# wavelab/libwave

Hardware: AMD Instinct MI355X
Metric: point-cloud registrations/sec (1M<->1M pts, ICP) (higher is better)
Workload: dtype f32

## Files before the change

include/wavematch.h:

```cpp
#ifndef WAVEMATCH_H
#define WAVEMATCH_H

#include <stddef.h>
#include <stdint.h>

#ifdef __cplusplus
extern "C" {
#endif

#define WM_OK 0
#define WM_NOT_CONVERGED 1
#define WM_TOO_FEW_CORRESPONDENCES 2
#define WM_ERR_ARG (-1)
#define WM_ERR_HIP (-2)
#define WM_ERR_RCCL (-3)
#define WM_ERR_STATE (-4)
#define WM_ERR_NOMEM (-5)

enum { WM_MEM_HOST = 0, WM_MEM_DEVICE = 1 };

typedef struct wm_ctx wm_ctx;

int wm_ctx_create(wm_ctx **out, int device);
void wm_ctx_destroy(wm_ctx *ctx);
// ... 33 lines not shown
    int nn_method;
    int carry_state;
    int profile;
    int normal_k;
    int reject;
    double reject_ratio;
    double reject_factor;
    int reject_min_corr;
} wm_icp_params;

typedef struct {
    int converged;
    int iterations;
    int state;
    int n_corr;
    double mse;
    double prev_mse;
    float align_ms;
    float nn_ms;
    float coarse_ms;
    float stats_ms;
    float solve_ms;
    int nn_launches;
    int nn_levels;
    uint64_t deferred;
    float grid_cell;
    int owned_violations;
    int cert_launches;
    float nn_cert_ms;
    float plan_ms;
    float compact_ms;
    float index_ms;
    float iter_ms;
    float allreduce_ms;
    unsigned n_tgt_local, n_src_local;
    int rccl_ranks;
    int shard_attempts;
    int late_iterations;
    int late_launches;
    float late_ms;
    int exchange_in_kernel;
    int n_matched;
    float reject_d2;
} wm_icp_stats;

void wm_icp_default_params(wm_icp_params *p);

int wm_icp_align(wm_ctx *ctx, const wm_icp_params *p, double T_out[16], wm_icp_stats *stats);

int wm_icp_match(wm_ctx *ctx, const void *ref, size_t n_ref, const void *target, size_t n_target,
                 size_t stride_bytes, int mem, const wm_icp_params *p, float res,
                 int multiscale_steps, double T_out[16], wm_icp_stats *stats);

#define WM_BATCH_LDS_TARGET_POINTS 10000
#define WM_BATCH_MAX_TARGET_POINTS 65535
typedef struct {
    const void *src;
    size_t n_src;
    const void *target;
    size_t n_target;
} wm_batch_item;
int wm_icp_batch_match(wm_ctx *ctx, const wm_batch_item *items, int n_items, size_t stride_bytes,
                       int mem, const wm_icp_params *p, float res, int multiscale_steps,
                       int with_info, double *T_out, double *info_out, wm_icp_stats *stats,
                       int *status);

int wm_voxel_downsample_batch(wm_ctx *ctx, const wm_batch_item *items, int n_items, size_t stride_bytes,
                              int mem, float leaf, float *out_xyz, size_t cap_points, size_t *n_out);

int wm_voxel_downsample(wm_ctx *ctx, const void *pts, size_t n, size_t stride_bytes, int mem,
                        float leaf, void *out, size_t out_stride, int out_mem, size_t cap,
                        size_t *n_out);

int wm_transform_cloud(wm_ctx *ctx, const void *pts, size_t n, size_t stride_bytes, int mem,
                       const double T[16], void *out, size_t out_stride, int out_mem);

enum { WM_INFO_LUM = 0, WM_INFO_CENSI = 1, WM_INFO_LUMOLD = 2 };
int wm_icp_info(wm_ctx *ctx, int method, const double T_result[16], double lin_covar,
                double ang_covar, double max_corr, double info[36], int *degenerate);

int wm_debug_copy_bandwidth(wm_ctx *ctx, size_t bytes, int reps, double *gb_per_s);
int wm_debug_bins_sum(const double *x, size_t n, const unsigned *perm, double *out, long long limbs_out[3]);
int wm_debug_sort_pairs(wm_ctx *ctx, const void *keys, int key_bytes, size_t n, unsigned bits, unsigned *values_out);
int wm_debug_knn(wm_ctx *ctx, int which, int k, int32_t *idx_out, float *d2_out);
int wm_set_option(wm_ctx *ctx, const char *name, double value);
int wm_debug_cert_log(wm_ctx *ctx, int iterations, unsigned *out, int cap);
int wm_debug_cert_prof(wm_ctx *ctx, unsigned long long *out, int cap);
int wm_debug_pub_log(wm_ctx *ctx, unsigned long long *out, int cap);
int wm_get_iteration_times(wm_ctx *ctx, float *nn_ms, int cap);

int wm_debug_solve_cycles(wm_ctx *ctx, unsigned long long out[8]);
int wm_debug_cost_log(wm_ctx *ctx, int iterations, unsigned *out, size_t cap);
int wm_debug_phase_log(wm_ctx *ctx, unsigned long long *out, int iterations);

int wm_get_correspondences(wm_ctx *ctx, int32_t *match_idx, float *d2, size_t cap);

int wm_nn_search(wm_ctx *ctx, const double T[16], double max_corr, int nn_method,
                 int32_t *match_idx, float *d2, size_t cap, float *kernel_ms);

int wm_estimate_normals(wm_ctx *ctx, int which, int k, void *normals_out, int out_mem);

#define WM_STATS_LEN 32
int wm_icp_stats_for(wm_ctx *ctx, const double T[16], int mode, double stats[WM_STATS_LEN]);

int wm_debug_rank_select(wm_ctx *ctx, const float *vals, size_t n, size_t rank, float *out);

typedef struct { int n_matched, n_kept; float threshold_d2; int all_kept; } wm_icp_reject_result;
int wm_icp_reject(wm_ctx *ctx, const double T[16], int mode, int reject, double ratio, double factor, int min_corr,
                  wm_icp_reject_result *res, unsigned char *kept_out, double stats_out[WM_STATS_LEN]);

int wm_umeyama_from_stats(const double stats[WM_STATS_LEN], double Tk_out[16]);
int wm_gn6_from_stats(const double stats[WM_STATS_LEN], double Tk_out[16]);

typedef struct {
    int corr_rand;
    int max_iter;
    double r_eps;
    double t_eps;
    double max_corr;
    double gicp_epsilon;
    int max_inner;
    int force_iterations;
    int objective;
    int reserved;
} wm_gicp_params;
#define WM_GICP_OBJECTIVE_PCL_SUMS 0
#define WM_GICP_OBJECTIVE_STATISTICS 1

typedef struct {
    int converged, iterations, n_corr, inner_total, evaluations;
    double f_final;
    float fdf_kernel_ms;
    int served_evaluations;
} wm_gicp_stats;

void wm_gicp_default_params(wm_gicp_params *p);
int wm_gicp_align(wm_ctx *ctx, const wm_gicp_params *p, double T_out[16], wm_gicp_stats *stats);
int wm_gicp_match(wm_ctx *ctx, const void *ref, size_t n_ref, const void *target, size_t n_target,
                  size_t stride_bytes, int mem, const wm_gicp_params *p, float res, double T_out[16],
                  wm_gicp_stats *stats);
int wm_set_source_filtered(wm_ctx *ctx, const void *pts, size_t n, size_t stride_bytes, int mem, float leaf);
int wm_set_target_filtered(wm_ctx *ctx, const void *pts, size_t n, size_t stride_bytes, int mem, float leaf);
#define WM_GICP_BATCH_MAX_POINTS 100000
int wm_gicp_batch_match(wm_ctx *ctx, const wm_batch_item *items, int n_items, size_t stride_bytes, int mem,
                        const wm_gicp_params *p, float res, double *T_out, wm_gicp_stats *stats, int *status,
                        float *kernel_ms);
int wm_gicp_eval(wm_ctx *ctx, const wm_gicp_params *p, const double T_pair[16], const double x[6],
                 double *f, double g[6], int *n_pairs);
int wm_gicp_covariances(wm_ctx *ctx, int k, double eps, double *cov_source, double *cov_target);

typedef struct {
    double res;
    double step_size;
    double t_eps;
    int max_iter;
    double outlier_ratio;
    int skip_line_search;
    int pcl_d1_sign;
    int force_iterations;
} wm_ndt_params;

typedef struct {
    int converged, iterations, n_voxels, evaluations;
    double score;
    float deriv_kernel_ms;
    int model_builds;
// ... 173 lines not shown
```

libwave_amd/capi.py:

```python
import ctypes as C
import os

import numpy as np

_HERE = os.path.dirname(os.path.abspath(__file__))
LIB_PATH = os.path.join(_HERE, "libwavematch_hip.so")

WM_OK, WM_NOT_CONVERGED, WM_TOO_FEW = 0, 1, 2
WM_ERR_ARG, WM_ERR_HIP, WM_ERR_RCCL, WM_ERR_STATE, WM_ERR_NOMEM = -1, -2, -3, -4, -5
WM_NDT_BATCH_MAX_POINTS = 200000
WM_GICP_BATCH_MAX_POINTS = 100000
WM_BATCH_LDS_TARGET_POINTS = 10000
WM_BATCH_MAX_TARGET_POINTS = 65535
WM_GROUND_BATCH_MAX_KEYS = 0xFFFFFFFF
WM_GROUND_BATCH_MAX_POINTS = 0x7FFFFFF0
WM_MEM_HOST, WM_MEM_DEVICE = 0, 1
WM_ICP_SVD, WM_ICP_GN6, WM_ICP_PLANE = 0, 1, 2
WM_REJECT_NONE, WM_REJECT_TRIMMED, WM_REJECT_MEDIAN = 0, 1, 2
WM_NN_AUTO, WM_NN_GRID, WM_NN_BRUTE = 0, 1, 2
WM_NN_WARM = 0x100
WM_INFO_LUM, WM_INFO_CENSI, WM_INFO_LUMOLD = 0, 1, 2
WM_STATS_LEN = 32
CONV_NAMES = {0: "NOT_CONVERGED", 1: "ITERATIONS", 2: "TRANSFORM", 3: "ABS_MSE", 4: "REL_MSE",
              5: "NO_CORRESPONDENCES", 6: "FORCED", 7: "DEGENERATE"}
# ... 156 lines not shown
        L.wm_debug_pub_log.argtypes = [C.c_void_p, C.POINTER(C.c_uint64), C.c_int]
        L.wm_cloud_sizes.argtypes = [C.c_void_p, C.POINTER(C.c_size_t), C.POINTER(C.c_size_t)]
        L.wm_icp_default_params.argtypes = [C.POINTER(IcpParams)]
        L.wm_icp_default_params.restype = None
        L.wm_icp_align.argtypes = [C.c_void_p, C.POINTER(IcpParams), _dp, C.POINTER(IcpStats)]
        L.wm_icp_match.argtypes = [C.c_void_p, C.c_void_p, C.c_size_t, C.c_void_p, C.c_size_t,
                                   C.c_size_t, C.c_int, C.POINTER(IcpParams), C.c_float, C.c_int,
                                   _dp, C.POINTER(IcpStats)]
        L.wm_icp_batch_match.argtypes = [C.c_void_p, C.POINTER(BatchItem), C.c_int, C.c_size_t, C.c_int,
                                         C.POINTER(IcpParams), C.c_float, C.c_int, C.c_int, _dp, _dp,
                                         C.POINTER(IcpStats), C.POINTER(C.c_int)]
        L.wm_gicp_batch_match.argtypes = [C.c_void_p, C.POINTER(BatchItem), C.c_int, C.c_size_t, C.c_int,
                                          C.POINTER(GicpParams), C.c_float, _dp, C.POINTER(GicpStats),
                                          C.POINTER(C.c_int), C.POINTER(C.c_float)]
        L.wm_ndt_batch_match.argtypes = [C.c_void_p, C.POINTER(BatchItem), C.c_int, C.c_size_t, C.c_int,
                                         C.POINTER(NdtParams), _dp, C.POINTER(NdtStats), C.POINTER(C.c_int),
                                         C.POINTER(C.c_float)]
        L.wm_voxel_downsample_batch.argtypes = [C.c_void_p, C.POINTER(BatchItem), C.c_int, C.c_size_t, C.c_int,
                                                C.c_float, _fp, C.c_size_t, C.POINTER(C.c_size_t)]
        L.wm_voxel_downsample.argtypes = [C.c_void_p, C.c_void_p, C.c_size_t, C.c_size_t, C.c_int,
                                          C.c_float, C.c_void_p, C.c_size_t, C.c_int, C.c_size_t,
                                          C.POINTER(C.c_size_t)]
        L.wm_transform_cloud.argtypes = [C.c_void_p, C.c_void_p, C.c_size_t, C.c_size_t, C.c_int,
                                         _dp, C.c_void_p, C.c_size_t, C.c_int]
        L.wm_icp_info.argtypes = [C.c_void_p, C.c_int, _dp, C.c_double, C.c_double, C.c_double, _dp,
                                  C.POINTER(C.c_int)]
        L.wm_ctx_set_stream.argtypes = [C.c_void_p, C.c_void_p, C.c_int]
        L.wm_icp_shard_begin.argtypes = [C.c_void_p, C.POINTER(IcpParams), C.c_double, C.c_double,
                                         C.c_size_t]
        L.wm_icp_shard_local_stats.argtypes = [C.c_void_p, C.c_void_p]
        L.wm_icp_shard_apply.argtypes = [C.c_void_p, C.c_void_p]
        L.wm_icp_shard_poll.argtypes = [C.c_void_p, C.POINTER(C.c_int), _dp, C.POINTER(IcpStats)]
        L.wm_host_icp_create.argtypes = [C.POINTER(C.c_void_p), C.POINTER(IcpParams), C.c_size_t]
        L.wm_host_icp_destroy.argtypes = [C.c_void_p]
        L.wm_host_icp_destroy.restype = None
        L.wm_host_icp_apply.argtypes = [C.c_void_p, _dp]
        L.wm_host_icp_get.argtypes = [C.c_void_p, C.POINTER(C.c_int), _dp, C.POINTER(IcpStats)]
        L.wm_gicp_default_params.argtypes = [C.POINTER(GicpParams)]
        L.wm_gicp_default_params.restype = None
        L.wm_gicp_align.argtypes = [C.c_void_p, C.POINTER(GicpParams), _dp, C.POINTER(GicpStats)]
        L.wm_gicp_match.argtypes = [C.c_void_p, C.c_void_p, C.c_size_t, C.c_void_p, C.c_size_t,
                                    C.c_size_t, C.c_int, C.POINTER(GicpParams), C.c_float, _dp,
                                    C.POINTER(GicpStats)]
        L.wm_gicp_eval.argtypes = [C.c_void_p, C.POINTER(GicpParams), _dp, _dp, _dp, _dp,
                                   C.POINTER(C.c_int)]
        L.wm_gicp_covariances.argtypes = [C.c_void_p, C.c_int, C.c_double, _dp, _dp]
        L.wm_ndt_default_params.argtypes = [C.POINTER(NdtParams)]
        L.wm_ndt_default_params.restype = None
        L.wm_ndt_align.argtypes = [C.c_void_p, C.POINTER(NdtParams), _dp, C.POINTER(NdtStats)]
        L.wm_ndt_derivatives.argtypes = [C.c_void_p, C.POINTER(NdtParams), _dp, _dp, _dp, _dp,
                                         C.POINTER(C.c_int)]
        L.wm_ndt_set_shard.argtypes = [C.c_void_p, C.c_int, C.c_int, ALLREDUCE_FN, C.c_void_p]
        L.wm_get_iteration_times.argtypes = [C.c_void_p, _fp, C.c_int]
        L.wm_comm_get_unique_id.argtypes = [C.c_void_p]
        L.wm_comm_init_rank.argtypes = [C.POINTER(C.c_void_p), C.c_int, C.c_void_p, C.c_int, C.c_int]
        L.wm_comm_init_all.argtypes = [C.POINTER(C.c_void_p), C.POINTER(C.c_int), C.c_int]
        L.wm_comm_init_local.argtypes = [C.POINTER(C.c_void_p), C.c_int, C.c_int]
        L.wm_comm_destroy.argtypes = [C.c_void_p]
        L.wm_comm_destroy.restype = None
        L.wm_comm_rank.argtypes = [C.c_void_p]
        L.wm_comm_allreduce_probe.argtypes = [C.c_void_p, C.c_void_p, C.c_int, _dp]
        L.wm_comm_world.argtypes = [C.c_void_p]
        L.wm_comm_mailboxes.argtypes = [C.c_void_p]
        L.wm_comm_set_exchange_timeout_ms.argtypes = [C.c_void_p, C.c_int]
        L.wm_icp_align_sharded.argtypes = [C.c_void_p, C.c_void_p, C.c_void_p, C.c_size_t, C.c_void_p,
                                           C.c_size_t, C.c_size_t, C.c_int, C.POINTER(IcpParams), _dp,
                                           C.POINTER(IcpStats)]
        L.wm_ndt_set_comm.argtypes = [C.c_void_p, C.c_void_p]
        L.wm_ndt_build_model.argtypes = [C.c_void_p, C.c_double]
        L.wm_set_source_filtered.argtypes = [C.c_void_p, C.c_void_p, C.c_size_t, C.c_size_t, C.c_int, C.c_float]
        L.wm_set_target_filtered.argtypes = [C.c_void_p, C.c_void_p, C.c_size_t, C.c_size_t, C.c_int, C.c_float]
        L.wm_multi_create.argtypes = [C.POINTER(C.c_void_p), C.POINTER(C.c_int), C.c_int, C.c_int]
        L.wm_multi_destroy.argtypes = [C.c_void_p]
        L.wm_multi_destroy.restype = None
        L.wm_multi_size.argtypes = [C.c_void_p]
        L.wm_multi_icp_align.argtypes = [C.c_void_p, C.c_void_p, C.c_size_t, C.c_void_p, C.c_size_t,
                                         C.c_size_t, C.POINTER(IcpParams), _dp, C.POINTER(IcpStats)]
        L.wm_multi_icp_match.argtypes = [C.c_void_p, C.c_void_p, C.c_size_t, C.c_void_p, C.c_size_t,
                                         C.c_size_t, C.POINTER(IcpParams), C.c_float, C.c_int, _dp, C.POINTER(IcpStats)]
        L.wm_multi_icp_info.argtypes = [C.c_void_p, C.c_int, _dp, C.c_double, C.c_double, C.c_double, _dp,
                                        C.POINTER(C.c_int)]
        L.wm_debug_solve_cycles.argtypes = [C.c_void_p, C.POINTER(C.c_uint64)]
        L.wm_debug_sort_pairs.argtypes = [C.c_void_p, C.c_void_p, C.c_int, C.c_size_t, C.c_uint, C.c_void_p]
        L.wm_debug_knn.argtypes = [C.c_void_p, C.c_int, C.c_int, _ip, _fp]
        L.wm_debug_cost_log.argtypes = [C.c_void_p, C.c_int, C.c_void_p, C.c_size_t]
        L.wm_debug_phase_log.argtypes = [C.c_void_p, C.c_void_p, C.c_int]
        L.wm_get_correspondences.argtypes = [C.c_void_p, _ip, _fp, C.c_size_t]
        L.wm_nn_search.argtypes = [C.c_void_p, _dp, C.c_double, C.c_int, _ip, _fp, C.c_size_t, _fp]
        L.wm_icp_stats_for.argtypes = [C.c_void_p, _dp, C.c_int, _dp]
        L.wm_debug_rank_select.argtypes = [C.c_void_p, _fp, C.c_size_t, C.c_size_t, _fp]
        L.wm_icp_reject.argtypes = [C.c_void_p, _dp, C.c_int, C.c_int, C.c_double, C.c_double, C.c_int,
                                    C.POINTER(IcpRejectResult), C.c_void_p, _dp]
        L.wm_estimate_normals.argtypes = [C.c_void_p, C.c_int, C.c_int, C.c_void_p, C.c_int]
        L.wm_umeyama_from_stats.argtypes = [_dp, _dp]
        L.wm_gn6_from_stats.argtypes = [_dp, _dp]
        L.wm_ground_default_params.argtypes = [C.POINTER(GroundParams)]
        L.wm_ground_default_params.restype = None
        L.wm_ground_segment.argtypes = [C.c_void_p, C.c_void_p, C.c_size_t, C.c_size_t, C.c_int,
                                        C.POINTER(GroundParams), C.c_int, C.c_void_p, C.c_size_t, C.c_int,
                                        C.POINTER(C.c_size_t), C.c_void_p, C.POINTER(GroundStats)]
        L.wm_ground_segment_batch.argtypes = [C.c_void_p, C.POINTER(GroundScan), C.c_int, C.c_size_t, C.c_int,
                                              C.POINTER(GroundParams), C.c_int, C.c_void_p, C.c_size_t, C.c_void_p,
                                              C.c_size_t, C.c_int, C.POINTER(C.c_size_t), C.c_void_p,
                                              C.POINTER(GroundStats), C.POINTER(C.c_float)]
        L.wm_outlier_default_params.argtypes = [C.POINTER(OutlierParams)]
        L.wm_outlier_default_params.restype = None
        L.wm_outlier_filter.argtypes = [C.c_void_p, C.c_void_p, C.c_size_t, C.c_size_t, C.c_int, C.POINTER(OutlierParams),
                                        C.c_void_p, C.c_size_t, C.c_int, C.POINTER(C.c_size_t), C.c_void_p, C.c_void_p,
                                        C.c_void_p, C.POINTER(OutlierStats)]
        L.wm_cluster_default_params.argtypes = [C.POINTER(ClusterParams)]
        L.wm_cluster_default_params.restype = None
        L.wm_cluster_extract.argtypes = [C.c_void_p, C.c_void_p, C.c_size_t, C.c_size_t, C.c_int, C.POINTER(ClusterParams),
                                         C.c_void_p, C.c_void_p, C.c_size_t, C.c_void_p, C.c_size_t, C.c_int,
                                         C.POINTER(C.c_size_t), C.POINTER(C.c_size_t), C.POINTER(ClusterStats)]
        L.wm_cluster_extract_batch.argtypes = [C.c_void_p, C.POINTER(ClusterScan), C.c_int, C.c_size_t, C.c_int,
                                               C.POINTER(ClusterParams), C.c_void_p, C.c_void_p, C.c_size_t, C.c_void_p,
                                               C.c_size_t, C.c_void_p, C.c_size_t, C.c_int, C.POINTER(C.c_size_t),
                                               C.POINTER(C.c_size_t), C.POINTER(ClusterStats), C.POINTER(C.c_float)]
        _LIB = L
    return _LIB


def declared_symbols(header=None):
    import re
    inc = os.path.join(os.path.dirname(_HERE), "include")
    names = []
    for fn in sorted(os.listdir(inc)):
        if not fn.endswith(".h"):
            continue
        txt = open(os.path.join(inc, fn)).read()
        txt = re.sub(r"/\*.*?\*/", "", txt, flags=re.S)
        names += re.findall(r"\b(wm_[a-z0-9_]+)\s*\(", txt)
    return sorted(set(names))


def gicp_params(**kw):
    p = GicpParams()
    lib().wm_gicp_default_params(C.byref(p))
    for k, v in kw.items():
        if not hasattr(p, k):
            raise AttributeError(k)
        setattr(p, k, v)
    return p


def ndt_params(**kw):
    p = NdtParams()
    lib().wm_ndt_default_params(C.byref(p))
    for k, v in kw.items():
        if not hasattr(p, k):
            raise AttributeError(k)
        setattr(p, k, v)
    return p


def icp_params(**kw):
    p = IcpParams()
    lib().wm_icp_default_params(C.byref(p))
    for k, v in kw.items():
        if not hasattr(p, k):
            raise AttributeError(k)
        setattr(p, k, v)
    return p


def ground_params(params=None, **kw):
# ... 571 lines not shown

    def set_stream(self, stream_ptr, external=True):
        self._check(lib().wm_ctx_set_stream(self._h, C.c_void_p(stream_ptr), int(external)),
                    "wm_ctx_set_stream")

    def shard_begin(self, params, x_lo, x_hi, expect_owned_total=0):
        self._check(lib().wm_icp_shard_begin(self._h, C.byref(params), float(x_lo), float(x_hi),
                                             int(expect_owned_total)), "wm_icp_shard_begin")

    def shard_local_stats(self, dev_ptr):
        self._check(lib().wm_icp_shard_local_stats(self._h, C.c_void_p(dev_ptr)),
                    "wm_icp_shard_local_stats")

    def shard_apply(self, dev_ptr):
        self._check(lib().wm_icp_shard_apply(self._h, C.c_void_p(dev_ptr)), "wm_icp_shard_apply")

    def shard_poll(self):
        done = C.c_int(0)
        T = np.zeros((4, 4), np.float64)
        s = IcpStats()
        rc = self._check(lib().wm_icp_shard_poll(self._h, C.byref(done), T.ctypes.data_as(_dp),
                                                 C.byref(s)), "wm_icp_shard_poll")
        d = self._stats_dict(rc, T, s)
        d["T"] = T
        d["done"] = bool(done.value)
        return d

    def icp_align_sharded(self, comm, ref, target, params=None, **kw):
        p = params or icp_params(**kw)
        rp, rn, rs, rm, k1 = _cloud_arg(ref)
        tp, tn, ts, tm, k2 = _cloud_arg(target)
        if rs != ts or rm != tm:
            raise WmError("ref and target must share stride and memory space")
        T = np.zeros((4, 4), np.float64)
        s = IcpStats()
        rc = self._check(lib().wm_icp_align_sharded(self._h, comm.handle if comm is not None else None,
                                                    C.c_void_p(rp), rn, C.c_void_p(tp), tn, rs, rm,
                                                    C.byref(p), T.ctypes.data_as(_dp), C.byref(s)),
                         "wm_icp_align_sharded")
        return self._sharded_dict(rc, T, s)

    @staticmethod
    def _sharded_dict(rc, T, s):
        d = Context._stats_dict(rc, T, s)
        d["owned_violations"] = s.owned_violations
        for k in ("plan_ms", "compact_ms", "index_ms", "iter_ms", "allreduce_ms", "n_tgt_local", "n_src_local",
                  "rccl_ranks", "shard_attempts", "exchange_in_kernel"):
            d[k] = getattr(s, k)
        return d

    def allreduce_probe(self, comm, reps=50):
        out = C.c_double(0)
        self._check(lib().wm_comm_allreduce_probe(self._h, comm.handle, int(reps), C.byref(out)),
                    "wm_comm_allreduce_probe")
        return out.value

    def ndt_set_comm(self, comm):
        self._check(lib().wm_ndt_set_comm(self._h, comm.handle if comm is not None else None),
                    "wm_ndt_set_comm")

    def cost_log_arm(self, iterations):
        self._check(lib().wm_debug_cost_log(self._h, iterations, None, 0), "wm_debug_cost_log")

    def cost_log_fetch(self, iterations, n):
        buf = np.zeros((iterations, n), np.uint32)
        k = lib().wm_debug_cost_log(self._h, iterations, buf.ctypes.data_as(C.c_void_p), buf.size)
        if k < 0:
            raise WmError("wm_debug_cost_log: %d" % k)
        return buf[:k]

    def phase_log_fetch(self, iterations):
        buf = np.zeros((iterations, 8), np.uint64)
        k = lib().wm_debug_phase_log(self._h, buf.ctypes.data_as(C.c_void_p), iterations)
        return buf[:max(k, 0)]

    def sort_pairs(self, keys, bits):
        keys = np.ascontiguousarray(keys)
        assert keys.dtype in (np.uint32, np.uint64) and keys.ndim == 1
        out = np.zeros(keys.shape[0], np.uint32)
        self._check(lib().wm_debug_sort_pairs(self._h, keys.ctypes.data, keys.dtype.itemsize, keys.shape[0], int(bits),
                                              out.ctypes.data), "wm_debug_sort_pairs")
        return out

    def debug_knn(self, which, k):
        n = self.n_tgt if which == 1 else self.n_src
        idx = np.full((n, int(k)), -1, np.int32)
        d2 = np.zeros((n, int(k)), np.float32)
        rc = self._check(lib().wm_debug_knn(self._h, int(which), int(k), idx.ctypes.data_as(_ip), d2.ctypes.data_as(_fp)),
                         "wm_debug_knn")
        if rc != WM_OK:
            raise WmError("wm_debug_knn: %s" % lib().wm_strerror(rc).decode())
        return idx, d2

    def solve_cycles(self):
        buf = (C.c_uint64 * 8)()
        lib().wm_debug_solve_cycles(self._h, buf)
        return [int(v) for v in buf]

    def iteration_times(self, cap=1024):
        buf = np.zeros(cap, np.float32)
        n = lib().wm_get_iteration_times(self._h, buf.ctypes.data_as(_fp), cap)
        return buf[:n].copy()

    def correspondences(self):
        idx = np.empty(self.n_src, np.int32)
        d2 = np.empty(self.n_src, np.float32)
        self._check(lib().wm_get_correspondences(self._h, idx.ctypes.data_as(_ip),
                                                 d2.ctypes.data_as(_fp), self.n_src),
                    "wm_get_correspondences")
        return idx, d2

    def nn_search(self, T=None, max_corr=3.0, nn_method=WM_NN_AUTO, want=True, timed=False):
        T = np.ascontiguousarray(np.eye(4) if T is None else T, np.float64)
        idx = np.empty(self.n_src, np.int32) if want else None
        d2 = np.empty(self.n_src, np.float32) if want else None
        ms = C.c_float(0)
        self._check(lib().wm_nn_search(self._h, T.ctypes.data_as(_dp), float(max_corr),
                                       int(nn_method), idx.ctypes.data_as(_ip) if want else None,
                                       d2.ctypes.data_as(_fp) if want else None, self.n_src,
                                       C.byref(ms) if timed else None), "wm_nn_search")
        return (idx, d2, ms.value) if timed else (idx, d2)

    def icp_stats_for(self, T, mode=WM_ICP_SVD):
        T = np.ascontiguousarray(T, np.float64)
        st = np.zeros(WM_STATS_LEN, np.float64)
        self._check(lib().wm_icp_stats_for(self._h, T.ctypes.data_as(_dp), int(mode),
                                           st.ctypes.data_as(_dp)), "wm_icp_stats_for")
        return st

    def icp_reject(self, T, mode=WM_ICP_SVD, reject=WM_REJECT_TRIMMED, ratio=0.5, factor=1.0, min_corr=0, want_stats=True):
        T = np.ascontiguousarray(T, np.float64)
        r = IcpRejectResult()
        kept = np.zeros(max(self.n_src, 1), np.uint8)
        st = np.zeros(WM_STATS_LEN, np.float64)
        self._check(lib().wm_icp_reject(self._h, T.ctypes.data_as(_dp), int(mode), int(reject), float(ratio), float(factor),
                                        int(min_corr), C.byref(r), kept.ctypes.data_as(C.c_void_p),
                                        st.ctypes.data_as(_dp) if want_stats else None), "wm_icp_reject")
        return dict(n_matched=r.n_matched, n_kept=r.n_kept, threshold_d2=np.float32(r.threshold_d2), all_kept=bool(r.all_kept),
                    kept=kept[:self.n_src].astype(bool), stats=st if want_stats else None)

    def debug_rank_select(self, vals, rank):
        vals = np.ascontiguousarray(vals, np.float32)
        out = C.c_float(0)
        self._check(lib().wm_debug_rank_select(self._h, vals.ctypes.data_as(_fp), vals.shape[0], int(rank), C.byref(out)),
                    "wm_debug_rank_select")
        return np.float32(out.value)


class HostIcp:

    def __init__(self, params, expect_owned_total=0):
        self._h = C.c_void_p()
        rc = lib().wm_host_icp_create(C.byref(self._h), C.byref(params), int(expect_owned_total))
        if rc != WM_OK:
            raise WmError("wm_host_icp_create failed")

    def __del__(self):
        if getattr(self, "_h", None):
            lib().wm_host_icp_destroy(self._h)
            self._h = None

    def apply(self, stats):
        st = np.ascontiguousarray(stats, np.float64)
        assert st.size == WM_STATS_LEN
        lib().wm_host_icp_apply(self._h, st.ctypes.data_as(_dp))

# ... 127 lines not shown
```

libwave_amd/csrc/wm_grid.hip:

```cpp
#include <cstring>

#include <rocprim/rocprim.hpp>

#include "wm_internal.hpp"
#include "wm_sort.hpp"

#include <math.h>
#include <vector>
#include <string.h>

namespace wm {

__global__ void __launch_bounds__(kBlock) k_pack(const unsigned char *in, size_t n, size_t stride,
                                                  float4 *out) {
    size_t i = (size_t) blockIdx.x * kBlock + threadIdx.x;
    if (i >= n) return;
    const float *p = reinterpret_cast<const float *>(in + i * stride);
    float x = p[0], y = p[1], z = p[2];
    if (!(isfinite(x) && isfinite(y) && isfinite(z))) {
        x = y = z = __builtin_nanf("");
    }
    out[i] = make_float4(x, y, z, __uint_as_float((unsigned) i));
}

template <bool PACK>
__global__ void k_bbox(float4 *pts, size_t n, float *out, const unsigned char *raw, size_t rstride);

bool upload_begin_async(wm_ctx *ctx, const void *pts, size_t bytes) {
    if (!ctx->side_stream || bytes == 0) return false;
    hipPointerAttribute_t at;
    if (hipPointerGetAttributes(&at, pts) != hipSuccess) {
        (void) hipGetLastError();
        return false;
    }
    if (at.type != hipMemoryTypeHost) return false;
    DevBuf &stage = ctx->staging2;
    if (stage.cap < bytes) {
        if (hipStreamSynchronize(ctx->stream) != hipSuccess || stage.reserve(bytes) != hipSuccess) return false;
    }
    if (hipMemcpyAsync(stage.p, pts, bytes, hipMemcpyHostToDevice, ctx->side_stream) != hipSuccess) {
        (void) hipGetLastError();
        (void) hipStreamSynchronize(ctx->side_stream);
        return false;
    }
    return true;
}

int pack_cloud(wm_ctx *ctx, const void *pts, size_t n, size_t stride, int mem, float4 *out, int slot, bool staged,
               float *bbox_partials, unsigned *bbox_blocks) {
    if (bbox_blocks) {
        unsigned b = (unsigned) ((n + kBlock - 1) / kBlock);
        *bbox_blocks = b > (unsigned) kBboxBlocks ? (unsigned) kBboxBlocks : b;
    }
    if (n == 0) return WM_OK;
    const unsigned char *dptr = nullptr;
    if (mem == WM_MEM_HOST && staged) {
        WM_HIP(ctx, hipStreamSynchronize(ctx->side_stream));
        dptr = ctx->staging2.as<unsigned char>();
    } else if (mem == WM_MEM_HOST) {
        DevBuf &stage = slot == 1 ? ctx->staging2 : ctx->staging;
        if (slot != 1) WM_HIP(ctx, hipStreamSynchronize(ctx->stream));
        if (stage.cap < n * stride) {
            WM_HIP(ctx, hipStreamSynchronize(ctx->stream));
            WM_HIP(ctx, stage.reserve(n * stride));
        }
        WM_HIP(ctx, hipMemcpy(stage.p, pts, n * stride, hipMemcpyHostToDevice));
        dptr = stage.as<unsigned char>();
    } else {
        dptr = static_cast<const unsigned char *>(pts);
    }
    unsigned blocks = (unsigned) ((n + kBlock - 1) / kBlock);
    if (bbox_partials && bbox_blocks) {
        hipLaunchKernelGGL(HIP_KERNEL_NAME(k_bbox<true>), dim3(*bbox_blocks), dim3(kBlock), 0, ctx->stream, out, n, bbox_partials, dptr, stride);
        WM_HIP(ctx, hipGetLastError());
        return WM_OK;
    }
    hipLaunchKernelGGL(k_pack, dim3(blocks), dim3(kBlock), 0, ctx->stream, dptr, n, stride, out);
    WM_HIP(ctx, hipGetLastError());
    if (bbox_partials && bbox_blocks) return launch_bbox(ctx, out, n, bbox_partials, bbox_blocks);
    return WM_OK;
}

template <bool PACK>
__global__ void __launch_bounds__(kBlock) k_bbox(float4 *pts, size_t n, float *out, const unsigned char *raw, size_t rstride) {
    float lo[3] = {INFINITY, INFINITY, INFINITY}, hi[3] = {-INFINITY, -INFINITY, -INFINITY};
    unsigned cnt = 0;
// ... 297 lines not shown
        WM_HIP(ctx, ctx->bbox_buf.reserve(sizeof(unsigned) * kOccBlocks));
        hipLaunchKernelGGL(k_count_occupied, dim3(blocks), dim3(kBlock), 0, ctx->stream,
                           lvl->cell_start.as<unsigned>(), (size_t) ncells, ctx->bbox_buf.as<unsigned>());
        WM_TRY(fast_fetch(ctx, part, ctx->bbox_buf.p, sizeof(unsigned) * blocks));
        uint64_t occ = 0;
        for (unsigned b = 0; b < blocks; ++b) occ += part[b];
        *avg_occupancy = occ ? (double) n / occ : 0.0;
    }
    return WM_OK;
}

static uint64_t cells_of(const Bbox &bb, float h) {
    uint64_t c = 1;
    for (int d = 0; d < 3; ++d) c *= (uint64_t) floor(((double) bb.hi[d] - bb.lo[d]) / h) + 1;
    return c;
}

int build_call_grid(wm_ctx *ctx, const float4 *pts, size_t n, size_t n_finite, const Bbox &bb, float floor_h,
                    GridLevel *grid) {
    double vol = 1;
    for (int d = 0; d < 3; ++d) vol *= fmax((double) bb.hi[d] - bb.lo[d], 1e-3);
    float h = fmaxf((float) fmax(cbrt(vol / (double) n_finite) * 1.5, 1e-4), floor_h);
    const uint64_t cell_cap = ((uint64_t) 1 << 26) + 8 * (uint64_t) n;
    while (cells_of(bb, h) > cell_cap) h *= 1.26f;
    double occ = 0;
    WM_TRY(build_grid_level(ctx, pts, n, bb, h, grid, &occ));
    if (occ > 6.0 || (occ > 0 && occ < 1.5)) {
        float h2 = fmaxf((float) (h * sqrt(3.0 / occ)), floor_h);
        while (cells_of(bb, h2) > cell_cap) h2 *= 1.26f;
        if (h2 != h) WM_TRY(build_grid_level(ctx, pts, n, bb, h2, grid, nullptr));
    }
    return WM_OK;
}

__global__ void __launch_bounds__(kBlock) k_morton_keys(const float4 *pts, unsigned n, MortonKey key,
                                                         unsigned invalid, unsigned *keys,
                                                         unsigned *vals) {
    const unsigned i = blockIdx.x * kBlock + threadIdx.x;
    if (i >= n) return;
    const float4 p = pts[i];
    keys[i] = p.x == p.x ? key(p) : invalid;
    vals[i] = i;
}

__global__ void __launch_bounds__(kBlock) k_gather(const float4 *pts, const unsigned *vals,
                                                    unsigned n, float4 *out) {
    const unsigned j = blockIdx.x * kBlock + threadIdx.x;
    if (j < n) out[j] = pts[vals[j]];
}

int morton_sort(wm_ctx *ctx, const float4 *pts, size_t n, const Bbox &bb, size_t n_valid,
                float4 *out) {
    if (n == 0 || n_valid == 0) return WM_OK;
    int bits = (int) ceil(log2(cbrt((double) n)));
    if (bits < 3) bits = 3;
    if (bits > 8) bits = 8;
    const int cells = 1 << bits;
    float ext[3];
    for (int d = 0; d < 3; ++d) ext[d] = fmaxf(bb.hi[d] - bb.lo[d], 1e-6f);
    MortonKey key{bb.lo[0], bb.lo[1], bb.lo[2], cells / ext[0], cells / ext[1], cells / ext[2],
                  cells};
    WM_HIP(ctx, ctx->vg_idx.reserve(n * 4));
    WM_HIP(ctx, ctx->vg_idx2.reserve(n * 4));
    WM_HIP(ctx, ctx->vg_perm.reserve(n * 4));
    WM_HIP(ctx, ctx->vg_perm2.reserve(n * 4));
    unsigned *k1 = ctx->vg_idx.as<unsigned>(), *k2 = ctx->vg_idx2.as<unsigned>();
    unsigned *v1 = ctx->vg_perm.as<unsigned>(), *v2 = ctx->vg_perm2.as<unsigned>();
    const unsigned blocks = (unsigned) ((n + kBlock - 1) / kBlock);
    hipLaunchKernelGGL(k_morton_keys, dim3(blocks), dim3(kBlock), 0, ctx->stream, pts, (unsigned) n,
                       key, 1u << (3 * bits), k1, v1);
    size_t tmp_bytes = 0;
    WM_HIP(ctx, sort_pairs_low_bits(nullptr, tmp_bytes, k1, k2, v1, v2, n, 3 * bits + 1, ctx->stream,
                                    (size_t) ctx->tune_radix_min));
    WM_HIP(ctx, ctx->vg_tmp.reserve(tmp_bytes));
    WM_HIP(ctx, sort_pairs_low_bits(ctx->vg_tmp.p, tmp_bytes, k1, k2, v1, v2, n, 3 * bits + 1, ctx->stream,
                                    (size_t) ctx->tune_radix_min));
    const unsigned gblocks = (unsigned) ((n_valid + kBlock - 1) / kBlock);
    hipLaunchKernelGGL(k_gather, dim3(gblocks), dim3(kBlock), 0, ctx->stream, pts, v2,
                       (unsigned) n_valid, out);
    WM_HIP(ctx, hipGetLastError());
    return WM_OK;
}

__device__ __forceinline__ void child_run(const unsigned *fs, int fnx, int fny, int fnz, int X,
                                          int Y, int Z, int r, unsigned *s, unsigned *e) {
    const int y = 2 * Y + (r & 1), z = 2 * Z + (r >> 1);
    *s = *e = 0;
    if (y >= fny || z >= fnz) return;
    const size_t base = ((size_t) z * fny + y) * fnx;
    const int xa = 2 * X, xb = min(2 * X + 2, fnx);
    *s = fs[base + xa];
    *e = fs[base + xb];
}

__global__ void __launch_bounds__(kBlock)
    k_coarse_count(const unsigned *__restrict__ fs, int fnx, int fny, int fnz, int cnx, int cny,
                   size_t ncells, unsigned *__restrict__ counts) {
    const size_t c = (size_t) blockIdx.x * kBlock + threadIdx.x;
    if (c >= ncells) return;
    const int X = (int) (c % cnx), Y = (int) ((c / cnx) % cny), Z = (int) (c / ((size_t) cnx * cny));
    unsigned total = 0;
#pragma unroll
    for (int r = 0; r < 4; ++r) {
        unsigned s, e;
        child_run(fs, fnx, fny, fnz, X, Y, Z, r, &s, &e);
        total += e - s;
    }
    counts[c] = total;
}

__global__ void __launch_bounds__(kBlock)
    k_coarse_move(const unsigned *__restrict__ fs, const float4 *__restrict__ fpts, size_t fncells,
                  LinearKey key0, int shift, int fnx, int fny, int fnz, int cnx, int cny,
                  const unsigned *__restrict__ cs, float4 *__restrict__ out, size_t cncells) {
    const unsigned j = blockIdx.x * kBlock + threadIdx.x;
    if (j == 0) {
        const unsigned end = cs[(size_t) cncells];
        const float nanv = __builtin_nanf("");
#pragma unroll
        for (int u = 0; u < 4; ++u) out[end + u] = make_float4(nanv, nanv, nanv, __uint_as_float(kNoIdx));
    }
    if (j >= fs[fncells]) return;
    const float4 p = fpts[j];
    int x = min(max((int) floorf((p.x - key0.ox) * key0.inv_h), 0), key0.nx - 1) >> shift;
    int y = min(max((int) floorf((p.y - key0.oy) * key0.inv_h), 0), key0.ny - 1) >> shift;
    int z = min(max((int) floorf((p.z - key0.oz) * key0.inv_h), 0), key0.nz - 1) >> shift;
    const int X = x >> 1, Y = y >> 1, Z = z >> 1, r = (y & 1) + 2 * (z & 1);
    unsigned dst = cs[((size_t) Z * cny + Y) * cnx + X];
    for (int q = 0; q < r; ++q) {
        unsigned s, e;
        child_run(fs, fnx, fny, fnz, X, Y, Z, q, &s, &e);
        dst += e - s;
    }
    unsigned s, e;
    child_run(fs, fnx, fny, fnz, X, Y, Z, r, &s, &e);
    out[dst + (j - s)] = p;
}

static int derive_grid_level(wm_ctx *ctx, const GridLevel &fine, int fine_index, GridLevel *lvl,
                             size_t n) {
    const GridDev &f = fine.d;
    const int nx = (f.nx + 1) / 2, ny = (f.ny + 1) / 2, nz = (f.nz + 1) / 2;
    const uint64_t ncells = (uint64_t) nx * ny * nz;
    lvl->ncells = ncells;
    WM_HIP(ctx, lvl->pts.reserve((n + 4) * sizeof(float4)));
    WM_HIP(ctx, lvl->cell_start.reserve((ncells + 1) * sizeof(unsigned)));
    WM_HIP(ctx, ctx->counts.reserve(ncells * sizeof(unsigned)));
    unsigned *counts = ctx->counts.as<unsigned>();
    const unsigned blocks = (unsigned) ((ncells + kBlock - 1) / kBlock);
    hipLaunchKernelGGL(k_coarse_count, dim3(blocks), dim3(kBlock), 0, ctx->stream, f.cell_start, f.nx,
                       f.ny, f.nz, nx, ny, (size_t) ncells, counts);
    WM_TRY(exclusive_scan(ctx, counts, ncells, lvl->cell_start.as<unsigned>()));
    {
        const GridDev &g0 = ctx->levels[0].d;
        const LinearKey key0{g0.ox, g0.oy, g0.oz, g0.inv_h, g0.nx, g0.ny, g0.nz};
        const unsigned pblocks = (unsigned) ((n + kBlock - 1) / kBlock);
        hipLaunchKernelGGL(k_coarse_move, dim3(pblocks), dim3(kBlock), 0, ctx->stream, f.cell_start,
                           f.pts, (size_t) fine.ncells, key0, fine_index, f.nx, f.ny, f.nz, nx, ny,
                           lvl->cell_start.as<unsigned>(), lvl->pts.as<float4>(), (size_t) ncells);
    }
    WM_HIP(ctx, hipGetLastError());
    lvl->d = f;
    lvl->d.h = 2.0f * f.h;
    lvl->d.inv_h = 1.0f / lvl->d.h;
    lvl->d.nx = nx;
    lvl->d.ny = ny;
    lvl->d.nz = nz;
    lvl->d.pts = lvl->pts.as<float4>();
    lvl->d.cell_start = lvl->cell_start.as<unsigned>();
    lvl->built = true;
    return WM_OK;
}

static int build_level0(wm_ctx *ctx) {
    const float4 *pts = ctx->tgt_orig.as<float4>();
    const Bbox &bb = ctx->tgt_bbox;
    const size_t n = ctx->n_tgt_input;
    double ext[3], vol = 1;
    for (int d = 0; d < 3; ++d) {
        ext[d] = fmax((double) bb.hi[d] - bb.lo[d], 1e-3);
        vol *= ext[d];
    }
    const uint64_t kMaxCells = 96ull << 20;
    auto clamp_h = [&](double h) {
        for (;;) {
            int nx, ny, nz;
            grid_dims(bb, (float) h, &nx, &ny, &nz);
            if ((uint64_t) nx * ny * nz <= kMaxCells) return h;
            h *= 1.26;
        }
    };
    double h;
    if (ctx->grid_cell_override > 0) {
        h = clamp_h(ctx->grid_cell_override);
        return build_grid_level(ctx, pts, n, bb, (float) h, &ctx->levels[0], nullptr);
    }
    const double target_occ = 3.0;
    h = clamp_h(fmax(cbrt(vol / fmax((double) ctx->n_tgt, 1.0)) * 1.5, 1e-4));
    if (ctx->tuned_h > 0 && ctx->tuned_n > 0) {
        const double rn = (double) ctx->n_tgt / (double) ctx->tuned_n;
        const double rv = vol / ctx->tuned_vol;
        if (rn > 0.8 && rn < 1.25 && rv > 0.6 && rv < 1.6) h = clamp_h(ctx->tuned_h);
        if (rn > 0.9 && rn < 1.1 && rv > 0.8 && rv < 1.25 && ++ctx->tuned_uses < 16)
            return build_grid_level(ctx, pts, n, bb, (float) h, &ctx->levels[0], nullptr);
    }
    ctx->tuned_uses = 0;
    double occ = 0;
    for (int it = 0; it < 3; ++it) {
        WM_TRY(build_grid_level(ctx, pts, n, bb, (float) h, &ctx->levels[0], &occ));
        if (occ <= 0) break;
        if (occ > target_occ * 0.6 && occ < target_occ * 1.6) break;
        double scale = sqrt(target_occ / occ);
        if (scale > 4) scale = 4;
        if (scale < 0.25) scale = 0.25;
        double nh = clamp_h(h * scale);
        if (fabs(nh - h) < 0.05 * h) break;
        h = nh;
    }
    if (!ctx->levels[0].built || ctx->levels[0].d.h != (float) h)
        WM_TRY(build_grid_level(ctx, pts, n, bb, (float) h, &ctx->levels[0], nullptr));
    ctx->tuned_h = h;
    ctx->tuned_n = ctx->n_tgt;
    ctx->tuned_vol = vol;
    return WM_OK;
}

int ensure_levels(wm_ctx *ctx, double max_corr) {
    if (!ctx->levels[0].built) {
        WM_TRY(build_level0(ctx));
        ctx->n_levels = 1;
        ctx->levels_max_corr = -1;
    }
    if (ctx->levels_max_corr == max_corr) return WM_OK;
    const float4 *pts = ctx->tgt_orig.as<float4>();
    double h = ctx->levels[0].d.h;
    int L = 1;
    while (h < 0.2 * max_corr && L < kMaxLevels) {
        h *= 2.0;
        WM_TRY(derive_grid_level(ctx, ctx->levels[L - 1], L - 1, &ctx->levels[L], ctx->n_tgt_input));
        ++L;
    }
    (void) pts;
    ctx->n_levels = L;
    ctx->levels_max_corr = max_corr;
    LevelsDev host{};
    for (int l = 0; l < L; ++l) host.g[l] = ctx->levels[l].d;
    host.n = L;
    WM_HIP(ctx, ctx->d_levels.reserve(sizeof(LevelsDev)));
    LevelsDev *stage = (LevelsDev *) ((char *) pinned_scratch(ctx, 0) + (32u << 10));
    if (!ctx->h_scratch) return WM_ERR_HIP;
    *stage = host;
    WM_HIP(ctx, hipMemcpyAsync(ctx->d_levels.p, stage, sizeof(host), hipMemcpyHostToDevice,
                               ctx->stream));
    return WM_OK;
}

}

extern "C" int wm_debug_sort_pairs(wm_ctx *ctx, const void *keys, int key_bytes, size_t n, unsigned bits, unsigned *values_out) {
    using namespace wm;
    if (!ctx || (n > 0 && (!keys || !values_out)) || (key_bytes != 4 && key_bytes != 8) || bits > 8u * (unsigned) key_bytes ||
        n >= (size_t) 0xFFFF0000u)
        return WM_ERR_ARG;
    if (n == 0) return WM_OK;
    WM_HIP(ctx, hipSetDevice(ctx->device));
    struct Scoped : DevBuf {
        ~Scoped() { release(); }
    } k1, k2, v1, v2, tmp;
    WM_HIP(ctx, k1.reserve(n * (size_t) key_bytes));
    WM_HIP(ctx, k2.reserve(n * (size_t) key_bytes));
    WM_HIP(ctx, v1.reserve(n * 4));
    WM_HIP(ctx, v2.reserve(n * 4));
    WM_HIP(ctx, tmp.reserve(rs_temp_bytes(n)));
    std::vector<unsigned> iota(n);
    for (size_t i = 0; i < n; ++i) iota[i] = (unsigned) i;
    WM_HIP(ctx, hipMemcpy(k1.p, keys, n * (size_t) key_bytes, hipMemcpyHostToDevice));
    WM_HIP(ctx, hipMemcpy(v1.p, iota.data(), n * 4, hipMemcpyHostToDevice));
    if (key_bytes == 4)
        WM_HIP(ctx, rs_sort_pairs(tmp.p, k1.as<unsigned>(), k2.as<unsigned>(), v1.as<unsigned>(), v2.as<unsigned>(), n, bits, ctx->stream));
    else
        WM_HIP(ctx, rs_sort_pairs(tmp.p, k1.as<unsigned long long>(), k2.as<unsigned long long>(), v1.as<unsigned>(), v2.as<unsigned>(), n,
                                  bits, ctx->stream));
    WM_HIP(ctx, hipStreamSynchronize(ctx->stream));
    WM_HIP(ctx, hipMemcpy(values_out, v2.p, n * 4, hipMemcpyDeviceToHost));
    return WM_OK;
}
```

Before: 274.4.

## Derive all coarse grid levels in two fused ladder kernels

Replaces the per-level count, exclusive scan and move sequence with two launches that handle every coarse level at once. Cell starts for each level are computed directly from the level-0 prefix array by summing row differences, with 64-lane wavefront reductions used for deep levels, so no scan is needed. A single move kernel then walks each point up the ladder, placing it at every level. This removes several kernel launches and scans per level build, at the cost of more redundant reads of the level-0 cell-start array in the starts kernel.

```diff
diff --git a/include/wavematch.h b/include/wavematch.h
--- a/include/wavematch.h
+++ b/include/wavematch.h
@@ -139,6 +139,7 @@
 int wm_debug_copy_bandwidth(wm_ctx *ctx, size_t bytes, int reps, double *gb_per_s);
 int wm_debug_bins_sum(const double *x, size_t n, const unsigned *perm, double *out, long long limbs_out[3]);
 int wm_debug_sort_pairs(wm_ctx *ctx, const void *keys, int key_bytes, size_t n, unsigned bits, unsigned *values_out);
+int wm_debug_grid_level(wm_ctx *ctx, int level, int dims_out[3], unsigned *cell_start_out, float *pts_out, size_t pts_cap);
 int wm_debug_knn(wm_ctx *ctx, int which, int k, int32_t *idx_out, float *d2_out);
 int wm_set_option(wm_ctx *ctx, const char *name, double value);
 int wm_debug_cert_log(wm_ctx *ctx, int iterations, unsigned *out, int cap);
diff --git a/libwave_amd/capi.py b/libwave_amd/capi.py
--- a/libwave_amd/capi.py
+++ b/libwave_amd/capi.py
@@ -262,6 +262,7 @@
                                         C.POINTER(C.c_int)]
         L.wm_debug_solve_cycles.argtypes = [C.c_void_p, C.POINTER(C.c_uint64)]
         L.wm_debug_sort_pairs.argtypes = [C.c_void_p, C.c_void_p, C.c_int, C.c_size_t, C.c_uint, C.c_void_p]
+        L.wm_debug_grid_level.argtypes = [C.c_void_p, C.c_int, C.POINTER(C.c_int), C.c_void_p, C.c_void_p, C.c_size_t]
         L.wm_debug_knn.argtypes = [C.c_void_p, C.c_int, C.c_int, _ip, _fp]
         L.wm_debug_cost_log.argtypes = [C.c_void_p, C.c_int, C.c_void_p, C.c_size_t]
         L.wm_debug_phase_log.argtypes = [C.c_void_p, C.c_void_p, C.c_int]
@@ -999,6 +1000,16 @@
                                               out.ctypes.data), "wm_debug_sort_pairs")
         return out
 
+    def grid_level(self, level):
+        dims = (C.c_int * 3)()
+        n_levels = self._check(lib().wm_debug_grid_level(self._h, int(level), dims, None, None, 0), "wm_debug_grid_level")
+        ncells = int(dims[0]) * int(dims[1]) * int(dims[2])
+        cs = np.zeros(ncells + 1, np.uint32)
+        pts = np.zeros((self.n_tgt + 4, 4), np.float32)
+        self._check(lib().wm_debug_grid_level(self._h, int(level), dims, cs.ctypes.data, pts.ctypes.data, pts.shape[0]),
+                    "wm_debug_grid_level")
+        return n_levels, (int(dims[0]), int(dims[1]), int(dims[2])), cs, pts[:int(cs[-1]) + 4]
+
     def debug_knn(self, which, k):
         n = self.n_tgt if which == 1 else self.n_src
         idx = np.full((n, int(k)), -1, np.int32)
diff --git a/libwave_amd/csrc/wm_grid.hip b/libwave_amd/csrc/wm_grid.hip
--- a/libwave_amd/csrc/wm_grid.hip
+++ b/libwave_amd/csrc/wm_grid.hip
@@ -2,6 +2,7 @@
 
 #include <rocprim/rocprim.hpp>
 
+#include "wm_grid_ladder.hpp"
 #include "wm_internal.hpp"
 #include "wm_sort.hpp"
 
@@ -465,93 +466,110 @@
     return WM_OK;
 }
 
-__device__ __forceinline__ void child_run(const unsigned *fs, int fnx, int fny, int fnz, int X,
-                                          int Y, int Z, int r, unsigned *s, unsigned *e) {
-    const int y = 2 * Y + (r & 1), z = 2 * Z + (r >> 1);
-    *s = *e = 0;
-    if (y >= fny || z >= fnz) return;
-    const size_t base = ((size_t) z * fny + y) * fnx;
-    const int xa = 2 * X, xb = min(2 * X + 2, fnx);
-    *s = fs[base + xa];
-    *e = fs[base + xb];
-}
-
-__global__ void __launch_bounds__(kBlock)
-    k_coarse_count(const unsigned *__restrict__ fs, int fnx, int fny, int fnz, int cnx, int cny,
-                   size_t ncells, unsigned *__restrict__ counts) {
-    const size_t c = (size_t) blockIdx.x * kBlock + threadIdx.x;
-    if (c >= ncells) return;
-    const int X = (int) (c % cnx), Y = (int) ((c / cnx) % cny), Z = (int) (c / ((size_t) cnx * cny));
-    unsigned total = 0;
+struct LadderDev {
+    int n_levels;
+    int nx, ny, nz;
+    const unsigned *fs;
+    const float4 *fpts;
+    unsigned *cs[kMaxLevels];
+    float4 *pts[kMaxLevels];
+    unsigned first_block[kMaxLevels + 1];
+};
+
+__global__ void __launch_bounds__(kBlock) k_ladder_starts(const LadderDev d) {
+    int L = 1;
+    unsigned first = d.first_block[1];
+    unsigned *cs = d.cs[1];
 #pragma unroll
-    for (int r = 0; r < 4; ++r) {
-        unsigned s, e;
-        child_run(fs, fnx, fny, fnz, X, Y, Z, r, &s, &e);
-        total += e - s;
-    }
-    counts[c] = total;
-}
-
-__global__ void __launch_bounds__(kBlock)
-    k_coarse_move(const unsigned *__restrict__ fs, const float4 *__restrict__ fpts, size_t fncells,
-                  LinearKey key0, int shift, int fnx, int fny, int fnz, int cnx, int cny,
-                  const unsigned *__restrict__ cs, float4 *__restrict__ out, size_t cncells) {
-    const unsigned j = blockIdx.x * kBlock + threadIdx.x;
-    if (j == 0) {
-        const unsigned end = cs[(size_t) cncells];
+    for (int l = 2; l < kMaxLevels; ++l)
+        if (l < d.n_levels && blockIdx.x >= d.first_block[l]) L = l, first = d.first_block[l], cs = d.cs[l];
+    const int lanes = ladder_lanes(L);
+    const size_t t = (size_t) (blockIdx.x - first) * kBlock + threadIdx.x;
+    const size_t c = lanes == 1 ? t : t >> 6;
+    const int lane = lanes == 1 ? 0 : (int) (t & 63);
+    const int cnx = ladder_dim(d.nx, L), cny = ladder_dim(d.ny, L), cnz = ladder_dim(d.nz, L);
+    const size_t ncells = (size_t) cnx * cny * cnz;
+    if (c > ncells) return;
+    unsigned s;
+    if (c == ncells) {
+        s = lane == 0 ? d.fs[(size_t) d.nx * d.ny * d.nz] : 0u;
+    } else {
+        const int X = (int) (c % cnx), Y = (int) ((c / cnx) % cny), Z = (int) (c / ((size_t) cnx * cny));
+        s = ladder_start_part(d.fs, d.nx, d.ny, d.nz, L, X, Y, Z, lane, lanes);
+    }
+    if (lanes != 1)
+        for (int off = 32; off > 0; off >>= 1) s += __shfl_down(s, off);
+    if (lane == 0) cs[c] = s;
+}
+
+__global__ void __launch_bounds__(kBlock) k_ladder_move(const LadderDev d, LinearKey key0) {
+    const unsigned j0 = blockIdx.x * kBlock + threadIdx.x;
+    const unsigned total = d.fs[(size_t) d.nx * d.ny * d.nz];
+    if (j0 == 0) {
         const float nanv = __builtin_nanf("");
 #pragma unroll
-        for (int u = 0; u < 4; ++u) out[end + u] = make_float4(nanv, nanv, nanv, __uint_as_float(kNoIdx));
-    }
-    if (j >= fs[fncells]) return;
-    const float4 p = fpts[j];
-    int x = min(max((int) floorf((p.x - key0.ox) * key0.inv_h), 0), key0.nx - 1) >> shift;
-    int y = min(max((int) floorf((p.y - key0.oy) * key0.inv_h), 0), key0.ny - 1) >> shift;
-    int z = min(max((int) floorf((p.z - key0.oz) * key0.inv_h), 0), key0.nz - 1) >> shift;
-    const int X = x >> 1, Y = y >> 1, Z = z >> 1, r = (y & 1) + 2 * (z & 1);
-    unsigned dst = cs[((size_t) Z * cny + Y) * cnx + X];
-    for (int q = 0; q < r; ++q) {
-        unsigned s, e;
-        child_run(fs, fnx, fny, fnz, X, Y, Z, q, &s, &e);
-        dst += e - s;
-    }
-    unsigned s, e;
-    child_run(fs, fnx, fny, fnz, X, Y, Z, r, &s, &e);
-    out[dst + (j - s)] = p;
-}
-
-static int derive_grid_level(wm_ctx *ctx, const GridLevel &fine, int fine_index, GridLevel *lvl,
-                             size_t n) {
-    const GridDev &f = fine.d;
-    const int nx = (f.nx + 1) / 2, ny = (f.ny + 1) / 2, nz = (f.nz + 1) / 2;
-    const uint64_t ncells = (uint64_t) nx * ny * nz;
-    lvl->ncells = ncells;
-    WM_HIP(ctx, lvl->pts.reserve((n + 4) * sizeof(float4)));
-    WM_HIP(ctx, lvl->cell_start.reserve((ncells + 1) * sizeof(unsigned)));
-    WM_HIP(ctx, ctx->counts.reserve(ncells * sizeof(unsigned)));
-    unsigned *counts = ctx->counts.as<unsigned>();
-    const unsigned blocks = (unsigned) ((ncells + kBlock - 1) / kBlock);
-    hipLaunchKernelGGL(k_coarse_count, dim3(blocks), dim3(kBlock), 0, ctx->stream, f.cell_start, f.nx,
-                       f.ny, f.nz, nx, ny, (size_t) ncells, counts);
-    WM_TRY(exclusive_scan(ctx, counts, ncells, lvl->cell_start.as<unsigned>()));
-    {
-        const GridDev &g0 = ctx->levels[0].d;
-        const LinearKey key0{g0.ox, g0.oy, g0.oz, g0.inv_h, g0.nx, g0.ny, g0.nz};
-        const unsigned pblocks = (unsigned) ((n + kBlock - 1) / kBlock);
-        hipLaunchKernelGGL(k_coarse_move, dim3(pblocks), dim3(kBlock), 0, ctx->stream, f.cell_start,
-                           f.pts, (size_t) fine.ncells, key0, fine_index, f.nx, f.ny, f.nz, nx, ny,
-                           lvl->cell_start.as<unsigned>(), lvl->pts.as<float4>(), (size_t) ncells);
-    }
+        for (int L = 1; L < kMaxLevels; ++L)
+            if (L < d.n_levels)
+                for (int u = 0; u < 4; ++u) d.pts[L][(size_t) total + u] = make_float4(nanv, nanv, nanv, __uint_as_float(kNoIdx));
+    }
+    if (j0 >= total) return;
+    const float4 p = d.fpts[j0];
+    int x = min(max((int) floorf((p.x - key0.ox) * key0.inv_h), 0), key0.nx - 1);
+    int y = min(max((int) floorf((p.y - key0.oy) * key0.inv_h), 0), key0.ny - 1);
+    int z = min(max((int) floorf((p.z - key0.oz) * key0.inv_h), 0), key0.nz - 1);
+    unsigned j = j0;
+    const unsigned *fs = d.fs;
+    int fnx = d.nx, fny = d.ny, fnz = d.nz;
+#pragma unroll
+    for (int L = 1; L < kMaxLevels; ++L) {
+        if (L >= d.n_levels) break;
+        const int cnx = (fnx + 1) / 2, cny = (fny + 1) / 2, cnz = (fnz + 1) / 2;
+        j = ladder_slot(fs, fnx, fny, fnz, d.cs[L], cnx, cny, x, y, z, j);
+        d.pts[L][j] = p;
+        fs = d.cs[L];
+        fnx = cnx, fny = cny, fnz = cnz;
+        x >>= 1, y >>= 1, z >>= 1;
+    }
+}
+
+static int derive_ladder(wm_ctx *ctx, int n_levels, size_t n) {
+    const GridLevel &l0 = ctx->levels[0];
+    const GridDev &g0 = l0.d;
+    LadderDev d{};
+    d.n_levels = n_levels;
+    d.nx = g0.nx, d.ny = g0.ny, d.nz = g0.nz;
+    d.fs = g0.cell_start;
+    d.fpts = g0.pts;
+    uint64_t blocks = 0;
+    for (int L = 1; L < n_levels; ++L) {
+        GridLevel *lvl = &ctx->levels[L];
+        const int nx = ladder_dim(g0.nx, L), ny = ladder_dim(g0.ny, L), nz = ladder_dim(g0.nz, L);
+        const uint64_t ncells = (uint64_t) nx * ny * nz;
+        lvl->ncells = ncells;
+        WM_HIP(ctx, lvl->pts.reserve((n + 4) * sizeof(float4)));
+        WM_HIP(ctx, lvl->cell_start.reserve((ncells + 1) * sizeof(unsigned)));
+        const GridDev &f = ctx->levels[L - 1].d;
+        lvl->d = f;
+        lvl->d.h = 2.0f * f.h;
+        lvl->d.inv_h = 1.0f / lvl->d.h;
+        lvl->d.nx = nx;
+        lvl->d.ny = ny;
+        lvl->d.nz = nz;
+        lvl->d.pts = lvl->pts.as<float4>();
+        lvl->d.cell_start = lvl->cell_start.as<unsigned>();
+        lvl->built = true;
+        d.cs[L] = lvl->cell_start.as<unsigned>();
+        d.pts[L] = lvl->pts.as<float4>();
+        d.first_block[L] = (unsigned) blocks;
+        blocks += ((ncells + 1) * (uint64_t) ladder_lanes(L) + kBlock - 1) / kBlock;
+    }
+    d.first_block[n_levels] = (unsigned) blocks;
+    if (n_levels < 2) return WM_OK;
+    hipLaunchKernelGGL(k_ladder_starts, dim3((unsigned) blocks), dim3(kBlock), 0, ctx->stream, d);
+    const LinearKey key0{g0.ox, g0.oy, g0.oz, g0.inv_h, g0.nx, g0.ny, g0.nz};
+    const unsigned pblocks = (unsigned) ((n + kBlock - 1) / kBlock);
+    hipLaunchKernelGGL(k_ladder_move, dim3(pblocks > 0 ? pblocks : 1u), dim3(kBlock), 0, ctx->stream, d, key0);
     WM_HIP(ctx, hipGetLastError());
-    lvl->d = f;
-    lvl->d.h = 2.0f * f.h;
-    lvl->d.inv_h = 1.0f / lvl->d.h;
-    lvl->d.nx = nx;
-    lvl->d.ny = ny;
-    lvl->d.nz = nz;
-    lvl->d.pts = lvl->pts.as<float4>();
-    lvl->d.cell_start = lvl->cell_start.as<unsigned>();
-    lvl->built = true;
     return WM_OK;
 }
 
@@ -615,15 +633,13 @@
         ctx->levels_max_corr = -1;
     }
     if (ctx->levels_max_corr == max_corr) return WM_OK;
-    const float4 *pts = ctx->tgt_orig.as<float4>();
     double h = ctx->levels[0].d.h;
     int L = 1;
     while (h < 0.2 * max_corr && L < kMaxLevels) {
         h *= 2.0;
-        WM_TRY(derive_grid_level(ctx, ctx->levels[L - 1], L - 1, &ctx->levels[L], ctx->n_tgt_input));
         ++L;
     }
-    (void) pts;
+    WM_TRY(derive_ladder(ctx, L, ctx->n_tgt_input));
     ctx->n_levels = L;
     ctx->levels_max_corr = max_corr;
     LevelsDev host{};
@@ -668,3 +684,22 @@
     WM_HIP(ctx, hipMemcpy(values_out, v2.p, n * 4, hipMemcpyDeviceToHost));
     return WM_OK;
 }
+
+extern "C" int wm_debug_grid_level(wm_ctx *ctx, int level, int dims_out[3], unsigned *cell_start_out, float *pts_out, size_t pts_cap) {
+    using namespace wm;
+    if (!ctx || level < 0 || !dims_out) return WM_ERR_ARG;
+    if (ctx->n_levels < 1 || !ctx->levels[0].built) return WM_ERR_STATE;
+    if (level >= ctx->n_levels) return WM_ERR_ARG;
+    WM_HIP(ctx, hipSetDevice(ctx->device));
+    WM_HIP(ctx, hipStreamSynchronize(ctx->stream));
+    const GridLevel &l = ctx->levels[level];
+    dims_out[0] = l.d.nx, dims_out[1] = l.d.ny, dims_out[2] = l.d.nz;
+    unsigned total = 0;
+    WM_HIP(ctx, hipMemcpy(&total, l.d.cell_start + l.ncells, sizeof(unsigned), hipMemcpyDeviceToHost));
+    if (cell_start_out) WM_HIP(ctx, hipMemcpy(cell_start_out, l.d.cell_start, (l.ncells + 1) * sizeof(unsigned), hipMemcpyDeviceToHost));
+    if (pts_out) {
+        if (pts_cap < (size_t) total + 4) return WM_ERR_ARG;
+        WM_HIP(ctx, hipMemcpy(pts_out, l.d.pts, ((size_t) total + 4) * sizeof(float4), hipMemcpyDeviceToHost));
+    }
+    return ctx->n_levels;
+}
diff --git a/libwave_amd/csrc/wm_grid_ladder.hpp b/libwave_amd/csrc/wm_grid_ladder.hpp
--- /dev/null
+++ b/libwave_amd/csrc/wm_grid_ladder.hpp
@@ -0,0 +1,58 @@
+#pragma once
+#include <stddef.h>
+
+#include "wm_math.hpp"
+
+namespace wm {
+
+WM_HD int ladder_dim(int n0, int L) { return ((n0 - 1) >> L) + 1; }
+
+WM_HD int ladder_lanes(int L) { return L >= 3 ? 64 : 1; }
+
+WM_HD unsigned ladder_start_part(const unsigned *fs, int fnx, int fny, int fnz, int L, int X, int Y, int Z, int lane,
+                                 int nlanes) {
+    const int B = 1 << L;
+    const int z0 = Z << L, y0 = Y << L;
+    const int z1 = z0 + B < fnz ? z0 + B : fnz, y1 = y0 + B < fny ? y0 + B : fny;
+    const size_t row = (size_t) fnx, slab = (size_t) fny * fnx, xo = (size_t) X << L;
+    unsigned s = lane == 0 ? fs[(size_t) z0 * slab] : 0u;
+    for (int z = z0 + lane; z < z1; z += nlanes) s += fs[(size_t) z * slab + (size_t) y0 * row] - fs[(size_t) z * slab];
+    const int rows = y1 - y0;
+    int z = z0 + lane / rows, y = y0 + lane % rows;
+    while (z < z1) {
+        const size_t b = (size_t) z * slab + (size_t) y * row;
+        s += fs[b + xo] - fs[b];
+        y += nlanes;
+        while (y >= y1) {
+            y -= rows;
+            ++z;
+        }
+    }
+    return s;
+}
+
+WM_HD void ladder_child_run(const unsigned *fs, int fnx, int fny, int fnz, int X, int Y, int Z, int r, unsigned *s,
+                            unsigned *e) {
+    const int y = 2 * Y + (r & 1), z = 2 * Z + (r >> 1);
+    *s = *e = 0;
+    if (y >= fny || z >= fnz) return;
+    const size_t base = ((size_t) z * fny + y) * fnx;
+    const int xa = 2 * X, xb = 2 * X + 2 < fnx ? 2 * X + 2 : fnx;
+    *s = fs[base + xa];
+    *e = fs[base + xb];
+}
+
+WM_HD unsigned ladder_slot(const unsigned *fs, int fnx, int fny, int fnz, const unsigned *cs, int cnx, int cny, int x, int y,
+                           int z, unsigned j) {
+    const int X = x >> 1, Y = y >> 1, Z = z >> 1, r = (y & 1) + 2 * (z & 1);
+    unsigned dst = cs[((size_t) Z * cny + Y) * cnx + X];
+    unsigned s, e;
+    for (int q = 0; q < r; ++q) {
+        ladder_child_run(fs, fnx, fny, fnz, X, Y, Z, q, &s, &e);
+        dst += e - s;
+    }
+    ladder_child_run(fs, fnx, fny, fnz, X, Y, Z, r, &s, &e);
+    return dst + (j - s);
+}
+
+}
```

Result: no change. 272.9 (-0.5%).
